# netocg/vae-decode-hdr

Hardware: NVIDIA B200
Metric: flux_vae_hdr_decode_megapixels_per_s (higher is better)
Workload: dtype fp16

## Files before the change

### vae_decode_hdr_b200/csrc/api.cu

```cuda
#include <stdarg.h>
#include <string.h>

#include <algorithm>
#include <functional>
#include <map>
#include <string>
#include <vector>

#include "engine.cuh"

namespace hdrvae {

static thread_local std::string g_last_error;
long long g_launch_count = 0;
void set_error(const char* fmt, ...) {
  char buf[1024];
  va_list ap;
  va_start(ap, fmt);
  vsnprintf(buf, sizeof buf, fmt, ap);
  va_end(ap);
  g_last_error = buf;
}

bool g_prof_on = false;
// ... 301 lines not shown
static bool x_is_16bit(hdrvae_ctx* ctx) {
  static int on = -1;
  if (on < 0) { const char* e = getenv("HDRVAE_X16"); on = (e && atoi(e) == 0) ? 0 : 1; }
  static int nin_on = -1;
  if (nin_on < 0) { const char* e = getenv("HDRVAE_FUSE_NIN"); nin_on = (e && atoi(e) == 0) ? 0 : 1; }
  return on && nin_on && !ctx->high && ctx->op_dtype == DT_F16 && ctx->conv_impl == HDRVAE_CONV_TCGEN05 && h_is_16bit(ctx);
}

static bool gn_is_fused(hdrvae_ctx* ctx, const PackedConv& pc, const ConvIO& io, int x_dtype, int H, int W) {
  static int on = -1;
  if (on < 0) {
    const char* e = getenv("HDRVAE_FUSE_GN");
    const char* g = getenv("HDRVAE_CTA_GROUP");
    on = ((e && atoi(e) == 0) || (g && atoi(g) == 1)) ? 0 : 1;
  }
  return on && x_is_16bit(ctx) && x_dtype == DT_F16 && pc.w_dtype == DT_F16 && pc.kmul == 1 && !pc.upsample && pc.ks == 3 &&
         pc.cout_pad >= 256 && pc.cin_pad % 64 == 0 && ctx->cta_group != 1 && io.x2 == nullptr && io.y_dtype == DT_F16 &&
         io.stats != nullptr && conv_takes_slab(pc, io, H, W, ctx->conv_impl);
}

static float* stats_ptr(hdrvae_ctx* ctx, DecState* st) {
  return ctx->conv_impl == HDRVAE_CONV_TCGEN05 ? reinterpret_cast<float*>(st->gn) : nullptr;
}

static int gn_before_conv(hdrvae_ctx* ctx, const void* x, const NormW& nw, const PackedConv& pc, ConvIO* io, DecState* st,
                          int B, int H, int W, cudaStream_t s, int x_dtype = DT_F32, float x_scale = 1.f) {
  if (gn_is_fused(ctx, pc, *io, x_dtype, H, W)) {
    char pname[64];
    snprintf(pname, sizeof pname, "groupnorm statistics C=%d @%dx%d", nw.C, B, H * W);
    ProfScope prof(pname, 0.0, 0.0, s);
    const int partials = st->pending;
    st->pending = 0;
    const float* scale = nullptr; const float* shift = nullptr;
// ... 10 lines not shown
  const int impl = ctx->conv_impl;
  const bool h16 = h_is_16bit(ctx);
  const int h_dt = h16 ? ctx->op_dtype : DT_F32;
  const float h_scale = h16 ? kRawOperandScale : 1.f;
  {
    ConvIO io; io.y = st->hbuf; io.stats = stats_ptr(ctx, st); io.stats_chunks = &st->pending;
    io.y_dtype = h_dt; io.y_scale = h_scale;
    HDRVAE_TRY(gn_before_conv(ctx, st->x, rw.n1, rw.c1, &io, st, B, H, W, s, st->x_dt, 1.f / st->x_scale));
    HDRVAE_TRY(run_conv(ctx, rw.c1, io, B, H, W, impl, s));
  }
  const bool x16 = st->x_dt != DT_F32;
  ConvIO io; io.stats = stats_ptr(ctx, st); io.stats_chunks = &st->pending;
  if (x16) { io.y_dtype = st->x_dt; io.y_scale = st->x_scale; }
  else if (rw.dual_out) { io.y2 = st->xa16; io.y2_dtype = ctx->op_dtype; io.y2_scale = kRawOperandScale; }
  if (rw.has_nin) {
    HDRVAE_TRY(run_gn(ctx, st->hbuf, h_dt, st->t, B, H * W, rw.n2, true, st, s, -1, 1.f / h_scale));
    io.x = st->t;
    if (nin_is_fused(ctx, rw, H, W)) {
      io.x2 = st->xb16; io.pc2 = &rw.nin_x16; io.bias = rw.bias_c2_nin; io.y = st->x;
      if (x16) {
        io.x2 = st->x; io.y = st->hbuf;
        HDRVAE_TRY(run_conv(ctx, rw.c2, io, B, H, W, impl, s));
        std::swap(st->x, st->hbuf);
        return 0;
      }
      return run_conv(ctx, rw.c2, io, B, H, W, impl, s);
    }
    HDRVAE_REQUIRE(!x16, "the 16-bit residual stream needs the fused shortcut");
    ConvIO sc; sc.x = st->xb16; sc.y = st->hbuf; sc.alpha = 1.0f / kRawOperandScale;
    HDRVAE_TRY(run_conv(ctx, rw.nin, sc, B, H, W, impl, s));
    io.y = st->hbuf; io.residual = st->hbuf;
    HDRVAE_TRY(run_conv(ctx, rw.c2, io, B, H, W, impl, s));
    std::swap(st->x, st->hbuf);
  } else {
    io.y = st->x; io.residual = st->x;
    if (x16) { io.res_dtype = st->x_dt; io.res_scale = 1.f / st->x_scale; }
    HDRVAE_TRY(gn_before_conv(ctx, st->hbuf, rw.n2, rw.c2, &io, st, B, H, W, s, h_dt, 1.f / h_scale));
    HDRVAE_TRY(run_conv(ctx, rw.c2, io, B, H, W, impl, s));
  }
  return 0;
// ... 145 lines not shown
    float* part = ksp > 1 ? reinterpret_cast<float*>(ksplit_scratch) : nullptr;
    return launch_attention_fused(q, 1024, (long long)pl.Tp * 1024, pl.T, q + 512, 1024, (long long)pl.Tp * 1024, pl.Tp, vt, pl.Tp,
                                  (long long)512 * pl.Tp, pl.T, o, (long long)pl.T * 512, pl.B, ctx->op_dtype, qk_alpha,
                                  attention_cta_group(ctx), ctx->num_sms, part, part ? part + (size_t)ksp * rows * 512 : nullptr,
                                  (long long)ksp * rows, s);
  }
  for (int b = 0; b < pl.B; ++b) {
    const uint16_t* q = reinterpret_cast<const uint16_t*>(qk) + (size_t)b * pl.Tp * 1024;
    HDRVAE_TRY(attention_rows(ctx, ws, pl.off_s, pl.off_p, pl.off_inv, pl.off_part, nullptr, 0, pl.s_rows, q, pl.T, q + 512,
                              reinterpret_cast<const uint16_t*>(vt) + (size_t)b * 512 * pl.Tp, pl.T, pl.Tp,
                              reinterpret_cast<uint16_t*>(o) + (size_t)b * pl.T * 512, qk_alpha, s));
  }
  return 0;
}

static int run_decoder(hdrvae_ctx* ctx, const float* latent, const Plan& pl, uint8_t* ws, void** features,
                       cudaStream_t s) {
  HDRVAE_REQUIRE(ctx->loaded, "hdrvae: weights not loaded");
  const int B = pl.B, impl = ctx->conv_impl, dt = ctx->op_dtype;
  int H = pl.h, W = pl.w;
  void* lat = ws + pl.off_lat;
  DecState st;
  st.xa16 = ws + pl.off_x16;
  st.xb16 = ws + pl.off_x16b;
  st.x = reinterpret_cast<float*>(ws + pl.off_x);
  st.hbuf = reinterpret_cast<float*>(ws + pl.off_h);
  st.t = ws + pl.off_t;
  st.gn = ws + pl.off_gn;
  st.gn_chunks = pl.gn_chunks;
  st.pending = 0;
  const bool x16 = x_is_16bit(ctx);
// ... 49 lines not shown
  HDRVAE_TRY(run_res(ctx, ctx->mid2, &st, B, H, W, s));
  for (int lvl = 3; lvl >= 0; --lvl) {
    for (int i = 0; i < 3; ++i) HDRVAE_TRY(run_res(ctx, ctx->up[lvl][i], &st, B, H, W, s));
    if (lvl != 0) {
      ConvIO io; io.x = st.xa16; io.y = st.hbuf; io.alpha = 1.0f / kRawOperandScale;
      if (x16) { io.x = st.x; io.y_dtype = st.x_dt; io.y_scale = st.x_scale; }
      else if (lvl <= 2) { io.y2 = st.xb16; io.y2_dtype = dt; io.y2_scale = kRawOperandScale; }
      io.stats = stats_ptr(ctx, &st); io.stats_chunks = &st.pending;
      HDRVAE_TRY(run_conv(ctx, ctx->upsample[lvl], io, B, H, W, impl, s));
      std::swap(st.x, st.hbuf);
      H *= 2; W *= 2;
    }
  }
  HDRVAE_TRY(run_gn(ctx, st.x, st.x_dt, st.t, B, H * W, ctx->norm_out, true, &st, s, ctx->high ? DT_F32 : -1, 1.f / st.x_scale));
  *features = st.t;
  return 0;
}

static int check_ws(const Plan& pl, void* ws, size_t bytes) {
  HDRVAE_REQUIRE(ws != nullptr && bytes >= pl.total, "hdrvae: workspace too small (%zu < %zu bytes)", bytes, pl.total);
  HDRVAE_REQUIRE((reinterpret_cast<uintptr_t>(ws) & 255) == 0, "hdrvae: workspace must be 256-byte aligned");
  return 0;
}


struct RowsPlan {
  int h, w, hl, world, T, Tl, Tp, s_rows, gn_chunks;
  size_t off_lat, off_x, off_h, off_t, off_xa, off_xb, off_gn, off_qk, off_v, off_vt, off_o, off_s, off_p, off_inv,
      off_part, off_epi, off_mail, total;
};
// ... 39 lines not shown

}

struct hdrvae_rows {
  hdrvae_ctx* ctx = nullptr;
  RowsPlan pl;
  int rank = 0, mode = 0;
  float factor = 1.f, ev = 1.f;
  uint8_t* ws = nullptr;
  const float* latent = nullptr;
  float* out = nullptr;
  struct Op { bool exchange; std::function<int(cudaStream_t)> fn; hdrvae_exchange ex; };
  std::vector<Op> ops;
  size_t pc = 0;
  float* x = nullptr; float* hbuf = nullptr;
  int H = 0, W = 0, pending = 0;
  uint8_t* peers[kRowsMaxRanks] = {};
  bool peers_set = false;
};

namespace hdrvae {

static void rows_compute(hdrvae_rows* st, std::function<int(cudaStream_t)> fn) {
  hdrvae_rows::Op op; op.exchange = false; op.fn = std::move(fn); memset(&op.ex, 0, sizeof op.ex);
  st->ops.push_back(std::move(op));
}
static void rows_exchange(hdrvae_rows* st, const hdrvae_exchange& ex) {
  hdrvae_rows::Op op; op.exchange = true; op.ex = ex;
  st->ops.push_back(std::move(op));
}
// ... 28 lines not shown
  hdrvae_exchange ex;
  memset(&ex, 0, sizeof ex);
  add_halo(st, &ex, slab_f32, H, W, C, eb);
  if (slab16 != nullptr) add_halo(st, &ex, slab16, H, W, C16, 2);
  ex.kind |= HDRVAE_EX_ALLREDUCE_F64;
  ex.allreduce_off = ws_off(st, gn_sums_ptr(gn, 1, 512, gn_chunks));
  ex.allreduce_count = 32 * 2;
  rows_exchange(st, ex);
  (void)ctx;
}

static void rows_gn(hdrvae_rows* st, const void* x_slab, const NormW& nw, bool silu, int H, int W, int x_dtype = DT_F32,
                    float in_scale = 1.f) {
  hdrvae_ctx* ctx = st->ctx;
  void* gn = st->ws + st->pl.off_gn;
  void* t = st->ws + st->pl.off_t;
  const int gn_chunks = st->pl.gn_chunks;
  const double count = (double)H * st->pl.world * (double)W * (double)(nw.C / 32);
  const NormW n = nw;
  rows_compute(st, [=](cudaStream_t s) {
    const long long slab = (long long)(H + 2) * W * n.C;
    HDRVAE_TRY(launch_gn_apply_from_sums(x_slab, x_dtype, slab, t, ctx->op_dtype, slab, 1, (H + 2) * W, n.C, n.gamma, n.beta,
                                         silu, gn, gn_chunks, count, s, in_scale));
    return zero_border_halos(st, t, H, W, n.C, 2, s);
  });
}

static void rows_res(hdrvae_rows* st, const ResW& rw, int H, int W) {
  hdrvae_ctx* ctx = st->ctx;
  void* t = st->ws + st->pl.off_t;
  void* xa = st->ws + st->pl.off_xa;
  void* xb = st->ws + st->pl.off_xb;
  float* stats = reinterpret_cast<float*>(st->ws + st->pl.off_gn);
  int* pending = &st->pending;
  float* x = st->x; float* hb = st->hbuf;
  const ResW* r = &rw;
  const bool h16 = h_is_16bit(ctx);
  const int h_dt = h16 ? ctx->op_dtype : DT_F32;
  const float h_scale = h16 ? kRawOperandScale : 1.f;
  const bool x16 = x_is_16bit(ctx);
  const int x_dt = x16 ? ctx->op_dtype : DT_F32;
  const float x_scale = x16 ? kRawOperandScale : 1.f;
  void* gn = st->ws + st->pl.off_gn;
  const int gn_chunks = st->pl.gn_chunks;
  const int y_lo = st->rank == 0 ? 0 : -1, y_hi = st->rank == st->pl.world - 1 ? H : H + 1;
// ... 1 lines not shown
  ConvIO probe1; probe1.y = hb; probe1.y_dtype = h_dt; probe1.stats = stats;
  const bool f1 = gn_is_fused(ctx, rw.c1, probe1, x_dt, H, W);
  if (!f1) rows_gn(st, x, rw.n1, true, H, W, x_dt, 1.f / x_scale);
  rows_compute(st, [=](cudaStream_t s) {
    ConvIO io; io.x = t; io.y = hb; io.stats = stats; io.stats_chunks = pending; io.x_pad = io.y_pad = 1;
    io.y_dtype = h_dt; io.y_scale = h_scale;
    if (f1) {
      HDRVAE_TRY(launch_gn_scale_shift_from_sums(1, r->n1.C, r->n1.gamma, r->n1.beta, gn, gn_chunks,
                                                 world_rows * (double)W * (double)(r->n1.C / 32), s, &io.xf_scale, &io.xf_shift));
      io.x = x; io.xf_in_scale = 1.f / x_scale; io.xf_y_lo = y_lo; io.xf_y_hi = y_hi;
    }
    return run_conv(ctx, r->c1, io, 1, H, W, HDRVAE_CONV_TCGEN05, s);
  });
  rows_stats_and_halo(st, hb, H, W, rw.c1.cout, nullptr, 0, h16 ? 2 : 4);
  const bool fused_nin = nin_is_fused(ctx, rw, H, W);
  float* out = (rw.has_nin && (!fused_nin || x16)) ? hb : x;
  ConvIO probe2; probe2.y = out; probe2.residual = rw.has_nin ? nullptr : out; probe2.y_dtype = x_dt; probe2.stats = stats;
  const bool f2 = !rw.has_nin && gn_is_fused(ctx, rw.c2, probe2, h_dt, H, W);
  if (!f2) rows_gn(st, hb, rw.n2, true, H, W, h_dt, 1.f / h_scale);
  rows_compute(st, [=](cudaStream_t s) {
    if (x16) {
      ConvIO io; io.x = t; io.y = out; io.stats = stats; io.stats_chunks = pending; io.x_pad = io.y_pad = 1;
      io.y_dtype = x_dt; io.y_scale = x_scale;
      if (fused_nin) { io.x2 = x; io.pc2 = &r->nin_x16; io.bias = r->bias_c2_nin; }
      else { io.residual = out; io.res_dtype = x_dt; io.res_scale = 1.f / x_scale; }
      if (f2) {
        HDRVAE_TRY(launch_gn_scale_shift_from_sums(1, r->n2.C, r->n2.gamma, r->n2.beta, gn, gn_chunks,
                                                   world_rows * (double)W * (double)(r->n2.C / 32), s, &io.xf_scale, &io.xf_shift));
        io.x = hb; io.xf_in_scale = 1.f / h_scale; io.xf_y_lo = y_lo; io.xf_y_hi = y_hi;
      }
      HDRVAE_TRY(run_conv(ctx, r->c2, io, 1, H, W, HDRVAE_CONV_TCGEN05, s));
      return zero_border_halos(st, out, H, W, r->c2.cout, 2, s);
    }
// ... 2 lines not shown
      io.x2 = xb; io.pc2 = &r->nin_x16; io.bias = r->bias_c2_nin;
      return run_conv(ctx, r->c2, io, 1, H, W, HDRVAE_CONV_TCGEN05, s);
    }
    if (r->has_nin) {
      ConvIO sc; sc.x = xb; sc.y = hb; sc.alpha = 1.0f / kRawOperandScale; sc.x_pad = sc.y_pad = 1;
      HDRVAE_TRY(run_conv(ctx, r->nin, sc, 1, H, W, HDRVAE_CONV_TCGEN05, s));
    }
    ConvIO io; io.x = t; io.y = out; io.residual = out; io.stats = stats; io.stats_chunks = pending; io.x_pad = io.y_pad = 1;
    if (r->dual_out) { io.y2 = xa; io.y2_dtype = ctx->op_dtype; io.y2_scale = kRawOperandScale; }
    HDRVAE_TRY(run_conv(ctx, r->c2, io, 1, H, W, HDRVAE_CONV_TCGEN05, s));
    if (r->dual_out) HDRVAE_TRY(zero_border_halos(st, xa, H, W, r->c2.cout, 2, s));
    return 0;
  });
  if (x16) rows_stats_and_halo(st, out, H, W, rw.c2.cout, nullptr, 0, 2);
  else rows_stats_and_halo(st, out, H, W, rw.c2.cout, rw.dual_out ? xa : nullptr, rw.c2.cout);
  if (rw.has_nin && (!fused_nin || x16)) std::swap(st->x, st->hbuf);
}

static int build_rows_program(hdrvae_rows* st) {
  hdrvae_ctx* ctx = st->ctx;
  const RowsPlan& pl = st->pl;
  const int dt = ctx->op_dtype;
  uint8_t* ws = st->ws;
  void* lat = ws + pl.off_lat;
  void* t = ws + pl.off_t;
  void* xa = ws + pl.off_xa;
  void* xb = ws + pl.off_xb;
  float* stats = reinterpret_cast<float*>(ws + pl.off_gn);
  int* pending = &st->pending;
  st->x = reinterpret_cast<float*>(ws + pl.off_x);
  st->hbuf = reinterpret_cast<float*>(ws + pl.off_h);
  int H = pl.hl, W = pl.w;
  const int rank = st->rank;
  const float* latent = st->latent;
  const bool x16 = x_is_16bit(ctx);
  const int x_dt = x16 ? dt : DT_F32;
  const float x_scale = x16 ? kRawOperandScale : 1.f;
  const int x_eb = x16 ? 2 : 4;

  {
    float* x = st->x;
    rows_compute(st, [=](cudaStream_t s) {
      HDRVAE_TRY(launch_latent_rows_to_nhwc(latent, lat, dt, 16, pl.h, pl.w, rank * pl.hl - 1, pl.hl + 2, 64, s));
      HDRVAE_TRY(gn_scratch_reset(stats, 1, pl.gn_chunks, s));
      ConvIO io; io.x = lat; io.y = x; io.stats = stats; io.stats_chunks = pending; io.x_pad = io.y_pad = 1;
      if (x16) { io.y_dtype = x_dt; io.y_scale = x_scale; }
      HDRVAE_TRY(run_conv(ctx, ctx->conv_in, io, 1, H, W, HDRVAE_CONV_TCGEN05, s));
      return x16 ? zero_border_halos(st, x, H, W, 512, 2, s) : 0;
    });
    rows_stats_and_halo(st, x, H, W, 512, nullptr, 0, x_eb);
  }
  rows_res(st, ctx->mid1, H, W);
  {
    uint16_t* qk = reinterpret_cast<uint16_t*>(ws + pl.off_qk);
    uint16_t* vb = reinterpret_cast<uint16_t*>(ws + pl.off_v);
    uint16_t* vt = reinterpret_cast<uint16_t*>(ws + pl.off_vt);
    uint16_t* o = reinterpret_cast<uint16_t*>(ws + pl.off_o);
    float* x = st->x;
    float* hscr = st->hbuf;
    const size_t hscr_bytes = (size_t)(8 * pl.hl + 2) * 8 * pl.w * 256 * 4;
    rows_gn(st, x, ctx->attn_norm, false, H, W, x_dt, 1.f / x_scale);
    rows_compute(st, [=](cudaStream_t s) {
      const uint16_t* tl = reinterpret_cast<const uint16_t*>(t) + (size_t)W * 512;
      if (pl.Tp != pl.T) {
        HDRVAE_CUDA_OK(cudaMemsetAsync(qk, 0, (size_t)pl.Tp * 1024 * 2, s));
        HDRVAE_CUDA_OK(cudaMemsetAsync(vt, 0, (size_t)512 * pl.Tp * 2, s));
      }
      HDRVAE_TRY(run_gemm(ctx, dt, tl, 512, pl.Tl, 512, ctx->qk.w[0], 512, 1024, 1024, qk + (size_t)rank * pl.Tl * 1024, 1024, dt,
                          ctx->qk.bias, false, 1.0f, nullptr, HDRVAE_CONV_TCGEN05, s));
      return run_gemm(ctx, dt, tl, 512, pl.Tl, 512, ctx->vproj.w[0], 512, 512, 512, vb + (size_t)rank * pl.Tl * 512, 512, dt,
                      ctx->vproj.bias, false, 1.0f, nullptr, HDRVAE_CONV_TCGEN05, s);
    });
    hdrvae_exchange ex;
    memset(&ex, 0, sizeof ex);
    ex.kind = HDRVAE_EX_ALLGATHER;
    ex.n_gather = 2;
// ... 22 lines not shown
        ConvIO io; io.x = xa; io.y = hb; io.alpha = 1.0f / kRawOperandScale; io.x_pad = io.y_pad = 1;
        if (x16) { io.x = xs; io.y_dtype = x_dt; io.y_scale = x_scale; }
        else if (lvl <= 2) { io.y2 = xb; io.y2_dtype = dt; io.y2_scale = kRawOperandScale; }
        io.stats = stats; io.stats_chunks = pending;
        HDRVAE_TRY(run_conv(ctx, *up, io, 1, Hc, Wc, HDRVAE_CONV_TCGEN05, s));
        return x16 ? zero_border_halos(st, hb, 2 * Hc, 2 * Wc, up->cout, 2, s) : 0;
      });
      H *= 2; W *= 2;
      rows_stats_and_halo(st, hb, H, W, up->cout, nullptr, 0, x_eb);
      std::swap(st->x, st->hbuf);
    }
  }
  {
    float* x = st->x;
    rows_gn(st, x, ctx->norm_out, true, H, W, x_dt, 1.f / x_scale);
    void* epi = ws + pl.off_epi;
    float* hscratch = st->hbuf;
    rows_compute(st, [=](cudaStream_t s) {
      return run_phase_a(ctx, t, 1, H, W, 1, hscratch, epi, s);
    });
    hdrvae_exchange ex;
    memset(&ex, 0, sizeof ex);
    ex.kind = HDRVAE_EX_RAW_STATS;
    ex.raw_stats_off = ws_off(st, epilogue_raw_stats_ptr(epi, 1, H, W));
    rows_exchange(st, ex);
    rows_compute(st, [=](cudaStream_t s) {
      return launch_epilogue_phase_b(1, H, W, st->mode, st->factor, st->ev, st->out, nullptr, epi, s);
    });
  }
  return 0;
// ... 248 lines not shown
  HDRVAE_CUDA_OK(cudaGraphLaunch(exec, s));
  return 0;
}

int hdrvae_decode_begin(hdrvae_ctx* ctx, const float* latent, int B, int h, int w, void* workspace, size_t ws_bytes,
                        void** raw_stats_dev, void* stream) {
  HDRVAE_REQUIRE(ctx != nullptr && latent != nullptr, "hdrvae_decode: null argument");
  HDRVAE_REQUIRE(B >= 1 && h >= 1 && w >= 1, "hdrvae_decode: empty latent batch [%d,16,%d,%d]", B, h, w);
  HDRVAE_CUDA_OK(cudaSetDevice(ctx->device));
  const Plan pl = make_plan(B, h, w, false, ctx->high, ctx->high || !attention_fused_enabled(ctx));
  HDRVAE_TRY(check_ws(pl, workspace, ws_bytes));
  uint8_t* ws = reinterpret_cast<uint8_t*>(workspace);
  cudaStream_t s = reinterpret_cast<cudaStream_t>(stream);
  auto body = [&](const float* lat) -> int {
    void* feat = nullptr;
    HDRVAE_TRY(run_decoder(ctx, lat, pl, ws, &feat, s));
    ProfScope prof("epilogue phase A (conv_out, max-pool, stats)", 2.0 * B * 64.0 * h * w * 3 * 1152, B * 64.0 * h * w * (256 + 24), s);
    return run_phase_a(ctx, feat, B, 8 * h, 8 * w, 0, reinterpret_cast<float*>(ws + pl.off_h), ws + pl.off_epi, s);
  };
  if (graphs_enabled(ctx, s)) {
    float* lat_in = reinterpret_cast<float*>(ws + pl.off_lat_in);
    HDRVAE_CUDA_OK(cudaMemcpyAsync(lat_in, latent, (size_t)B * 16 * pl.T * 4, cudaMemcpyDeviceToDevice, s));
    hdrvae_ctx::GraphEntry key{0, B, h, w, 0, ctx->conv_impl, ctx->cta_group, 0.f, 0.f, workspace, nullptr, 0};
    HDRVAE_TRY(run_segment(ctx, key, s, [&]() { return body(lat_in); }));
  } else {
    HDRVAE_TRY(body(latent));
  }
  if (raw_stats_dev != nullptr) *raw_stats_dev = epilogue_raw_stats_ptr(ws + pl.off_epi, B, 8 * h, 8 * w);
  return 0;
}

int hdrvae_decode_finish(hdrvae_ctx* ctx, int B, int h, int w, int mode, float expansion_factor, float ev_multiplier,
                         float* out_bhwc, hdrvae_stats* stats, void* workspace, size_t ws_bytes, void* stream) {
// ... 196 lines not shown
    if (e != cudaSuccess) { set_error("hdrvae_rows_end: %s", cudaGetErrorString(e)); r = -1; }
  }
  delete st;
  return r;
}

int hdrvae_decode_features(hdrvae_ctx* ctx, const float* latent, int B, int h, int w, void* features, void* workspace,
                           size_t ws_bytes, void* stream) {
  HDRVAE_REQUIRE(ctx != nullptr && latent != nullptr && features != nullptr, "hdrvae_decode_features: null argument");
  HDRVAE_REQUIRE(B >= 1 && h >= 1 && w >= 1, "hdrvae_decode_features: empty latent batch");
  HDRVAE_CUDA_OK(cudaSetDevice(ctx->device));
  const Plan pl = make_plan(B, h, w, false, ctx->high, ctx->high || !attention_fused_enabled(ctx));
  HDRVAE_TRY(check_ws(pl, workspace, ws_bytes));
  cudaStream_t s = reinterpret_cast<cudaStream_t>(stream);
  void* feat = nullptr;
  HDRVAE_TRY(run_decoder(ctx, latent, pl, reinterpret_cast<uint8_t*>(workspace), &feat, s));
  HDRVAE_CUDA_OK(cudaMemcpyAsync(features, feat, (size_t)B * 64 * h * w * 128 * (ctx->high ? 4 : 2), cudaMemcpyDeviceToDevice, s));
  return 0;
}

int hdrvae_epilogue_scratch_bytes(int B, int H, int W, size_t* bytes) {
  HDRVAE_REQUIRE(bytes != nullptr && B >= 1 && H >= 1 && W >= 1, "hdrvae_epilogue_scratch_bytes: bad argument");
  *bytes = epilogue_scratch_bytes(B, H, W);
  return 0;
}

int hdrvae_epilogue(hdrvae_ctx* ctx, const void* pre, int dtype, int B, int H, int W, const float* conv_w,
                    const float* conv_b, int mode, float expansion_factor, float ev_multiplier, float* out_bhwc,
                    hdrvae_stats* stats, float* dbg_post3, float* dbg_pre3, int32_t* dbg_argmax3, void* scratch,
                    size_t scratch_bytes, void* stream) {
  HDRVAE_REQUIRE(ctx != nullptr && pre != nullptr && conv_w != nullptr && conv_b != nullptr && out_bhwc != nullptr,
// ... 119 lines not shown
```

### vae_decode_hdr_b200/csrc/gemm_tc.cu

```cuda
#include "common.cuh"
#pragma nv_diag_suppress 128
#include "ptx.cuh"

#ifndef HDRVAE_SLAB_PITCH
#define HDRVAE_SLAB_PITCH 10
#endif

namespace hdrvae {

constexpr int kBlockM = 128;
constexpr int kRowBytes = 128;
constexpr int kABytes = kBlockM * kRowBytes;
constexpr int kEpilogueThreads = 256;
constexpr int kNumThreads = 128 + kEpilogueThreads;
constexpr int kRegsControl = 64, kRegsEpilogue = 216;

constexpr int kSmemLimit = 232448;
constexpr int kSmemFixed = 8 * 4096  + 256  +
                           1024 ;

constexpr int kSlabRows = 18, kSlabPitch = HDRVAE_SLAB_PITCH;
constexpr int kSlabBytes = kSlabRows * kSlabPitch * kRowBytes;
constexpr int kSlabBufBytes = (kSlabBytes + 1023) / 1024 * 1024;
template <int BLOCK_N, int CG, int KSUB, int SLAB = 0>
// ... 52 lines not shown
  EPI_GENERIC = 1,
  EPI_OUT16 = 2,
  EPI_RES = 4,
  EPI_OUT2 = 8,
  EPI_STATS = 16,
  EPI_ROWOPS = 32,
  EPI_LRELU = 64,
  EPI_RES2 = 128,
  EPI_ROWMAX = 256,
  EPI_EXPSUM = 512,
  EPI_RES16 = 1024,
};

constexpr int kXfWarps = 8;
constexpr int kXfThreads = kNumThreads + kXfWarps * 32;
constexpr int kRegsControlXf = 64, kRegsXf = 64, kRegsEpilogueXf = 144;

template <int BLOCK_N, bool kTf32, int CG, int EPI, int KSUB, int SLAB = 0, bool XF = false>
__global__ void __launch_bounds__(XF ? kXfThreads : kNumThreads, 1)
gemm_tc_kernel(const __grid_constant__ CUtensorMap tmA, const __grid_constant__ CUtensorMap tmB,
               const __grid_constant__ CUtensorMap tmA2, const __grid_constant__ CUtensorMap tmB2, const GemmParams p) {
  using Cfg = TcConfig<BLOCK_N, CG, KSUB, SLAB>;
  constexpr int kAT = Cfg::kATile;
  const uint32_t rank = CG == 2 ? ptx::cluster_ctarank() : 0u;
  constexpr int kStages = Cfg::kStages;
  constexpr int kActiveEpiWarps = BLOCK_N >= 64 ? 8 : 4;
  constexpr int kElemsPerRow = kTf32 ? 32 : 64;
  extern __shared__ uint8_t smem_raw[];
  uint8_t* smem = smem_raw + ((1024u - (ptx::smem_u32(smem_raw) & 1023u)) & 1023u);
  uint8_t* smem_a = smem;
  uint8_t* smem_b = SLAB ? smem : smem + kStages * KSUB * kAT;
// ... 39 lines not shown
  if (CG == 2) ptx::cluster_sync_all(); else __syncthreads();
  ptx::tc_fence_after_sync();
  const uint32_t tmem_base = *tmem_ptr_s;

  const int tiles_per_img = p.tiles_x * p.tiles_y;
  const int m_tiles = p.n_img * tiles_per_img;
  const int num_tiles = ((m_tiles + CG - 1) / CG) * p.n_tiles_n;
  const int w_first = blockIdx.x / CG, w_step = gridDim.x / CG;
  const int kb_per_tap = p.k_per_tap / kElemsPerRow;
  const int num_kb = p.ntaps * kb_per_tap;
  const int kb2_blocks = SLAB ? p.k2 / kElemsPerRow : 0;
  const int ntg = SLAB ? p.ntaps / SLAB : 0;
  constexpr bool xf = XF && SLAB > 0;

  const int num_groups = (num_kb + KSUB - 1) / KSUB;
  if (warp < 4 || warp >= 12) {
  if (!XF) ptx::reg_dec<kRegsControl>();
  else if (warp < 4) ptx::reg_dec<kRegsControlXf>();
  else ptx::reg_dec<kRegsXf>();
  if (warp == 0) {
    int stage = 0, ss = 0;
    uint32_t phase = 0, sphase = 0;
    int s_tile = w_first, s_kb = 0;
    auto issue_next_slab = [&]() {
      if (s_tile >= num_tiles) return;
      const int mt = (s_tile / p.n_tiles_n) * CG + (int)rank;
      const int img = mt / tiles_per_img;
      const int rem = mt - img * tiles_per_img;
      const int ty = rem / p.tiles_x;
      const int tx = rem - ty * p.tiles_x;
      const int x0 = tx * p.TW, y0 = ty * p.TH;
      ptx::mbar_wait(&slab_empty_bar[ss], sphase ^ 1);
      if (ptx::elect_one()) {
        uint8_t* sa = smem_slab + ss * Cfg::kSlabBuf;
// ... 207 lines not shown
            }
          }
          if (CG == 2) ptx::umma_commit_pair(&empty_bar[stage]); else ptx::umma_commit(&empty_bar[stage]);
          if (g == num_groups - 1) {
            if (CG == 2) ptx::umma_commit_pair(&tmem_full_bar[acc]); else ptx::umma_commit(&tmem_full_bar[acc]);
          }
        }
        __syncwarp();
        if (++stage == kStages) { stage = 0; phase ^= 1; }
      }
      if (++acc == 2) { acc = 0; acc_phase ^= 1; }
    }
    if (tim && blockIdx.x == 0 && lane == 0)
      printf("gemm_tc<%d,cg%d,epi%d,slab%d> issuer: %lld cycles, %d tiles x %d k-blocks; waited: accumulator %lld, slab %lld, B stage %lld\n",
             BLOCK_N, CG, EPI, SLAB, clock64() - t_begin, (num_tiles - w_first + w_step - 1) / w_step, num_kb, w_acc, w_slab, w_b);
  } else if (warp >= 12 && xf) {
    if constexpr (xf) {
      const int tl = (warp - 12) * 32 + lane;
      const int c = tl & 7, lg = tl >> 3;
      const uint32_t chunk_off = (uint32_t)((c ^ (lg & 7)) << 4);
      const int C = p.k_per_tap;
      const int y_hi = p.xf_y_hi;
      int ss = 0;
      uint32_t sphase = 0;
      const bool tim = (p.dbg & 32) != 0;
      long long w_land = 0, w_work = 0, tq = 0;
      for (int tile = w_first; tile < num_tiles; tile += w_step) {
        const int mt = (tile / p.n_tiles_n) * CG + (int)rank;
        const int img = mt / tiles_per_img;
        const int rem = mt - img * tiles_per_img;
        const int ty = rem / p.tiles_x;
        const int tx = rem - ty * p.tiles_x;
        const int x0 = tx * p.TW - 1, y0 = ty * p.TH - 1;
        const bool img_ok = img < p.n_img;
        for (int kb = 0; kb < kb_per_tap; ++kb) {
          float2 a2[4], b2[4];
#pragma unroll
          for (int e = 0; e < 4; ++e) {
            const int ch = kb * kElemsPerRow + c * 8 + 2 * e;
            const bool ok = img_ok && ch + 1 < C;
            a2[e].x = ok ? __ldg(p.xf_scale + (long long)img * C + ch) * p.xf_in_scale : 0.f;
            a2[e].y = ok ? __ldg(p.xf_scale + (long long)img * C + ch + 1) * p.xf_in_scale : 0.f;
            b2[e].x = ok ? __ldg(p.xf_shift + (long long)img * C + ch) : 0.f;
            b2[e].y = ok ? __ldg(p.xf_shift + (long long)img * C + ch + 1) : 0.f;
          }
          if (tim) tq = clock64();
          ptx::mbar_wait(&slab_full_bar[ss], sphase);
          if (tim) { const long long now = clock64(); w_land += now - tq; tq = now; }
          uint8_t* base = smem_slab + ss * Cfg::kSlabBuf + chunk_off;
          int r = lg / kSlabPitch, px = lg - r * kSlabPitch;
#pragma unroll 2
          for (int L = lg; L < kSlabRows * kSlabPitch; L += 32) {
            uint4* q = reinterpret_cast<uint4*>(base + L * kRowBytes);
            const int x = x0 + px, y = y0 + r;
            const bool inside = x >= 0 && x < p.W && y >= p.xf_y_lo && y < y_hi;
            uint4 v = *q;
            __half2* h = reinterpret_cast<__half2*>(&v);
#pragma unroll
            for (int e = 0; e < 4; ++e) {
              const float2 o = silu_nr2(f2_fma(__half22float2(h[e]), a2[e], b2[e]));
              h[e] = __floats2half2_rn(o.x, o.y);
            }
            if (!inside) v = make_uint4(0u, 0u, 0u, 0u);
            *q = v;
            px += 32 - 3 * kSlabPitch;
            r += 3;
            if (px >= kSlabPitch) { px -= kSlabPitch; ++r; }
          }
          ptx::fence_proxy_async();
          __syncwarp();
          if (lane == 0) {
            if (CG == 2) ptx::mbar_arrive_cluster(&slab_ready_bar[ss], 0);
            else ptx::mbar_arrive(&slab_ready_bar[ss]);
          }
          if (tim) w_work += clock64() - tq;
          if (++ss == Cfg::kSlabStages) { ss = 0; sphase ^= 1; }
        }
      }
      if (tim && blockIdx.x == 0 && warp == 12 && lane == 0)
        printf("gemm_tc<%d,cg%d,epi%d,slab%d> transform warp 0: waited for slabs to land %lld cycles, transformed them in %lld\n",
               BLOCK_N, CG, EPI, SLAB, w_land, w_work);
    }
// ... 653 lines not shown
      } else {
        epi = -1;
      }
    } else if (res16 && !p.round_tf32 && p.out_dtype == p.res_dtype && p.out2 == nullptr && !rowops && p.stats != nullptr) {
      epi = EPI_OUT16 | EPI_RES16 | EPI_STATS;
    } else {
      epi = -1;
    }
    if (p.row_mode != 0) {
      HDRVAE_REQUIRE(!n128 && p.tw_log2 == 7 && p.H == 1 && p.row_part != nullptr && p.ntaps == 1 && p.b_img_k_stride == 0,
                     "gemm_tc: the soft-max passes are row-major GEMMs with >= 256 columns");
      if (p.row_mode == 1) return launch_tc<256, false, 2, EPI_ROWMAX>(p, num_sms, stream);
      HDRVAE_REQUIRE(p.out_dtype != DT_F32 && p.bias != nullptr, "gemm_tc: soft-max pass 2 writes a 16-bit output and needs -max per row");
      return launch_tc<256, false, 2, EPI_OUT16 | EPI_EXPSUM>(p, num_sms, stream);
    }
    if (p.slab && n128 && p.ntaps == 9 && p.TW == 8 && p.TH == 16 && p.b_img_k_stride == 0) {
      if (epi == EPI_STATS) return launch_tc<128, false, 2, EPI_STATS, 3>(p, num_sms, stream);
      if (epi == (EPI_OUT16 | EPI_STATS)) return launch_tc<128, false, 2, EPI_OUT16 | EPI_STATS, 3>(p, num_sms, stream);
      if (epi == (EPI_RES | EPI_STATS)) return launch_tc<128, false, 2, EPI_RES | EPI_STATS, 3>(p, num_sms, stream);
      if (epi == (EPI_RES | EPI_OUT2 | EPI_STATS)) return launch_tc<128, false, 2, EPI_RES | EPI_OUT2 | EPI_STATS, 3>(p, num_sms, stream);
      if (epi == (EPI_OUT16 | EPI_RES16 | EPI_STATS)) return launch_tc<128, false, 2, EPI_OUT16 | EPI_RES16 | EPI_STATS, 3>(p, num_sms, stream);
      if (epi == 0) return launch_tc<128, false, 2, 0, 3>(p, num_sms, stream);
      if (epi == EPI_RES) return launch_tc<128, false, 2, EPI_RES, 3>(p, num_sms, stream);
    }
    if (p.slab && !n128 && p.ntaps == 4 && p.TW == 8 && p.TH == 16 && p.b_img_k_stride == 0) {
      if (epi == (EPI_OUT2 | EPI_STATS)) return launch_tc<256, false, 2, EPI_OUT2 | EPI_STATS, 1>(p, num_sms, stream);
      if (epi == EPI_STATS) return launch_tc<256, false, 2, EPI_STATS, 1>(p, num_sms, stream);
      if (epi == (EPI_OUT16 | EPI_STATS)) return launch_tc<256, false, 2, EPI_OUT16 | EPI_STATS, 1>(p, num_sms, stream);
      HDRVAE_REQUIRE(false, "gemm_tc: no slab build for this upsample epilogue (%d)", epi);
    }
    if (p.xf_scale != nullptr) {
      HDRVAE_REQUIRE(p.slab && !n128 && p.ntaps == 9 && p.TW == 8 && p.TH == 16 && p.b_img_k_stride == 0 && p.k2 == 0,
                     "gemm_tc: the fused GroupNorm exists for the 256-column 3x3 slab convs");
      if (epi == (EPI_OUT16 | EPI_STATS)) return launch_tc<256, false, 2, EPI_OUT16 | EPI_STATS, 1, true>(p, num_sms, stream);
      if (epi == (EPI_OUT16 | EPI_RES16 | EPI_STATS)) return launch_tc<256, false, 2, EPI_OUT16 | EPI_RES16 | EPI_STATS, 1, true>(p, num_sms, stream);
      HDRVAE_REQUIRE(false, "gemm_tc: no fused-GroupNorm build for this epilogue (%d)", epi);
    }
    if (p.slab && !n128 && p.ntaps == 9 && p.TW == 8 && p.TH == 16 && p.b_img_k_stride == 0) {
      if (epi == EPI_STATS) return launch_tc<256, false, 2, EPI_STATS, 1>(p, num_sms, stream);
      if (epi == (EPI_OUT16 | EPI_STATS)) return launch_tc<256, false, 2, EPI_OUT16 | EPI_STATS, 1>(p, num_sms, stream);
      if (epi == (EPI_RES | EPI_STATS)) return launch_tc<256, false, 2, EPI_RES | EPI_STATS, 1>(p, num_sms, stream);
      if (epi == (EPI_RES | EPI_OUT2 | EPI_STATS)) return launch_tc<256, false, 2, EPI_RES | EPI_OUT2 | EPI_STATS, 1>(p, num_sms, stream);
      if (epi == (EPI_OUT16 | EPI_RES16 | EPI_STATS)) return launch_tc<256, false, 2, EPI_OUT16 | EPI_RES16 | EPI_STATS, 1>(p, num_sms, stream);
    }
#define HDRVAE_EPI_CASE(E)                                                                       \
    case E:                                                                                      \
      return n128 ? launch_tc<128, false, 2, E>(p, num_sms, stream) : launch_tc<256, false, 2, E>(p, num_sms, stream);
    switch (epi) {
      HDRVAE_EPI_CASE(0)
      HDRVAE_EPI_CASE(EPI_RES)
      HDRVAE_EPI_CASE(EPI_STATS)
// ... 21 lines not shown
```

Baseline: 117.9.

## Extend fused GroupNorm to shortcut and 128-column convs, add interior slab fast path

Fused GroupNorm+SiLU-in-the-conv-prologue now also covers convs with a fused 1x1 shortcut (x2) and 128-column (n128) convs. This removes the standalone GroupNorm pass and its round trip through the t buffer in residual blocks with a channel-change shortcut. The t buffer is rotated to serve as an output, and the spare x buffer is passed to phase A as scratch. The transform warps gain an unrolled interior-tile path that skips per-pixel bounds logic, and register budgets are rebalanced between the transform and epilogue warps, at the cost of more template instantiations and register pressure.

```diff
diff --git a/vae_decode_hdr_b200/csrc/api.cu b/vae_decode_hdr_b200/csrc/api.cu
--- a/vae_decode_hdr_b200/csrc/api.cu
+++ b/vae_decode_hdr_b200/csrc/api.cu
@@ -339,9 +339,10 @@
     const char* g = getenv("HDRVAE_CTA_GROUP");
     on = ((e && atoi(e) == 0) || (g && atoi(g) == 1)) ? 0 : 1;
   }
+  const bool cols_ok = pc.cout_pad >= 256 || pc.cin_pad >= 256 || io.x2 != nullptr;
   return on && x_is_16bit(ctx) && x_dtype == DT_F16 && pc.w_dtype == DT_F16 && pc.kmul == 1 && !pc.upsample && pc.ks == 3 &&
-         pc.cout_pad >= 256 && pc.cin_pad % 64 == 0 && ctx->cta_group != 1 && io.x2 == nullptr && io.y_dtype == DT_F16 &&
-         io.stats != nullptr && conv_takes_slab(pc, io, H, W, ctx->conv_impl);
+         cols_ok && pc.cin_pad % 64 == 0 && ctx->cta_group != 1 && io.y_dtype == DT_F16 && io.stats != nullptr &&
+         conv_takes_slab(pc, io, H, W, ctx->conv_impl);
 }
 
 static float* stats_ptr(hdrvae_ctx* ctx, DecState* st) {
@@ -382,16 +383,20 @@
   if (x16) { io.y_dtype = st->x_dt; io.y_scale = st->x_scale; }
   else if (rw.dual_out) { io.y2 = st->xa16; io.y2_dtype = ctx->op_dtype; io.y2_scale = kRawOperandScale; }
   if (rw.has_nin) {
+    if (nin_is_fused(ctx, rw, H, W) && x16) {
+      io.x2 = st->x; io.pc2 = &rw.nin_x16; io.bias = rw.bias_c2_nin;
+      const bool gn_fused = gn_is_fused(ctx, rw.c2, io, h_dt, H, W);
+      HDRVAE_TRY(gn_before_conv(ctx, st->hbuf, rw.n2, rw.c2, &io, st, B, H, W, s, h_dt, 1.f / h_scale));
+      io.y = gn_fused ? st->t : st->hbuf;
+      HDRVAE_TRY(run_conv(ctx, rw.c2, io, B, H, W, impl, s));
+      if (gn_fused) { st->t = st->x; st->x = static_cast<float*>(io.y); }
+      else std::swap(st->x, st->hbuf);
+      return 0;
+    }
     HDRVAE_TRY(run_gn(ctx, st->hbuf, h_dt, st->t, B, H * W, rw.n2, true, st, s, -1, 1.f / h_scale));
     io.x = st->t;
     if (nin_is_fused(ctx, rw, H, W)) {
       io.x2 = st->xb16; io.pc2 = &rw.nin_x16; io.bias = rw.bias_c2_nin; io.y = st->x;
-      if (x16) {
-        io.x2 = st->x; io.y = st->hbuf;
-        HDRVAE_TRY(run_conv(ctx, rw.c2, io, B, H, W, impl, s));
-        std::swap(st->x, st->hbuf);
-        return 0;
-      }
       return run_conv(ctx, rw.c2, io, B, H, W, impl, s);
     }
     HDRVAE_REQUIRE(!x16, "the 16-bit residual stream needs the fused shortcut");
@@ -567,7 +572,7 @@
   return 0;
 }
 
-static int run_decoder(hdrvae_ctx* ctx, const float* latent, const Plan& pl, uint8_t* ws, void** features,
+static int run_decoder(hdrvae_ctx* ctx, const float* latent, const Plan& pl, uint8_t* ws, void** features, float** spare,
                        cudaStream_t s) {
   HDRVAE_REQUIRE(ctx->loaded, "hdrvae: weights not loaded");
   const int B = pl.B, impl = ctx->conv_impl, dt = ctx->op_dtype;
@@ -647,6 +652,7 @@
   }
   HDRVAE_TRY(run_gn(ctx, st.x, st.x_dt, st.t, B, H * W, ctx->norm_out, true, &st, s, ctx->high ? DT_F32 : -1, 1.f / st.x_scale));
   *features = st.t;
+  if (spare != nullptr) *spare = st.x;
   return 0;
 }
 
@@ -716,6 +722,7 @@
   std::vector<Op> ops;
   size_t pc = 0;
   float* x = nullptr; float* hbuf = nullptr;
+  void* t = nullptr;
   int H = 0, W = 0, pending = 0;
   uint8_t* peers[kRowsMaxRanks] = {};
   bool peers_set = false;
@@ -774,7 +781,7 @@
                     float in_scale = 1.f) {
   hdrvae_ctx* ctx = st->ctx;
   void* gn = st->ws + st->pl.off_gn;
-  void* t = st->ws + st->pl.off_t;
+  void* t = st->t;
   const int gn_chunks = st->pl.gn_chunks;
   const double count = (double)H * st->pl.world * (double)W * (double)(nw.C / 32);
   const NormW n = nw;
@@ -788,7 +795,7 @@
 
 static void rows_res(hdrvae_rows* st, const ResW& rw, int H, int W) {
   hdrvae_ctx* ctx = st->ctx;
-  void* t = st->ws + st->pl.off_t;
+  void* t = st->t;
   void* xa = st->ws + st->pl.off_xa;
   void* xb = st->ws + st->pl.off_xb;
   float* stats = reinterpret_cast<float*>(st->ws + st->pl.off_gn);
@@ -820,9 +827,12 @@
   });
   rows_stats_and_halo(st, hb, H, W, rw.c1.cout, nullptr, 0, h16 ? 2 : 4);
   const bool fused_nin = nin_is_fused(ctx, rw, H, W);
-  float* out = (rw.has_nin && (!fused_nin || x16)) ? hb : x;
-  ConvIO probe2; probe2.y = out; probe2.residual = rw.has_nin ? nullptr : out; probe2.y_dtype = x_dt; probe2.stats = stats;
-  const bool f2 = !rw.has_nin && gn_is_fused(ctx, rw.c2, probe2, h_dt, H, W);
+  ConvIO probe2; probe2.y_dtype = x_dt; probe2.stats = stats;
+  if (fused_nin && x16) probe2.x2 = x;
+  if (!rw.has_nin) probe2.residual = x;
+  const bool f2 = (!rw.has_nin || (fused_nin && x16)) && gn_is_fused(ctx, rw.c2, probe2, h_dt, H, W);
+  const bool rotate_t = rw.has_nin && f2;
+  void* out = rotate_t ? t : (rw.has_nin && (!fused_nin || x16)) ? static_cast<void*>(hb) : static_cast<void*>(x);
   if (!f2) rows_gn(st, hb, rw.n2, true, H, W, h_dt, 1.f / h_scale);
   rows_compute(st, [=](cudaStream_t s) {
     if (x16) {
@@ -855,7 +865,8 @@
   });
   if (x16) rows_stats_and_halo(st, out, H, W, rw.c2.cout, nullptr, 0, 2);
   else rows_stats_and_halo(st, out, H, W, rw.c2.cout, rw.dual_out ? xa : nullptr, rw.c2.cout);
-  if (rw.has_nin && (!fused_nin || x16)) std::swap(st->x, st->hbuf);
+  if (rotate_t) { st->t = st->x; st->x = static_cast<float*>(out); }
+  else if (rw.has_nin && (!fused_nin || x16)) std::swap(st->x, st->hbuf);
 }
 
 static int build_rows_program(hdrvae_rows* st) {
@@ -864,13 +875,13 @@
   const int dt = ctx->op_dtype;
   uint8_t* ws = st->ws;
   void* lat = ws + pl.off_lat;
-  void* t = ws + pl.off_t;
   void* xa = ws + pl.off_xa;
   void* xb = ws + pl.off_xb;
   float* stats = reinterpret_cast<float*>(ws + pl.off_gn);
   int* pending = &st->pending;
   st->x = reinterpret_cast<float*>(ws + pl.off_x);
   st->hbuf = reinterpret_cast<float*>(ws + pl.off_h);
+  st->t = ws + pl.off_t;
   int H = pl.hl, W = pl.w;
   const int rank = st->rank;
   const float* latent = st->latent;
@@ -901,6 +912,7 @@
     float* hscr = st->hbuf;
     const size_t hscr_bytes = (size_t)(8 * pl.hl + 2) * 8 * pl.w * 256 * 4;
     rows_gn(st, x, ctx->attn_norm, false, H, W, x_dt, 1.f / x_scale);
+    void* t = st->t;
     rows_compute(st, [=](cudaStream_t s) {
       const uint16_t* tl = reinterpret_cast<const uint16_t*>(t) + (size_t)W * 512;
       if (pl.Tp != pl.T) {
@@ -953,6 +965,7 @@
   {
     float* x = st->x;
     rows_gn(st, x, ctx->norm_out, true, H, W, x_dt, 1.f / x_scale);
+    void* t = st->t;
     void* epi = ws + pl.off_epi;
     float* hscratch = st->hbuf;
     rows_compute(st, [=](cudaStream_t s) {
@@ -1231,9 +1244,10 @@
   cudaStream_t s = reinterpret_cast<cudaStream_t>(stream);
   auto body = [&](const float* lat) -> int {
     void* feat = nullptr;
-    HDRVAE_TRY(run_decoder(ctx, lat, pl, ws, &feat, s));
+    float* conv8 = nullptr;
+    HDRVAE_TRY(run_decoder(ctx, lat, pl, ws, &feat, &conv8, s));
     ProfScope prof("epilogue phase A (conv_out, max-pool, stats)", 2.0 * B * 64.0 * h * w * 3 * 1152, B * 64.0 * h * w * (256 + 24), s);
-    return run_phase_a(ctx, feat, B, 8 * h, 8 * w, 0, reinterpret_cast<float*>(ws + pl.off_h), ws + pl.off_epi, s);
+    return run_phase_a(ctx, feat, B, 8 * h, 8 * w, 0, conv8, ws + pl.off_epi, s);
   };
   if (graphs_enabled(ctx, s)) {
     float* lat_in = reinterpret_cast<float*>(ws + pl.off_lat_in);
@@ -1460,7 +1474,7 @@
   HDRVAE_TRY(check_ws(pl, workspace, ws_bytes));
   cudaStream_t s = reinterpret_cast<cudaStream_t>(stream);
   void* feat = nullptr;
-  HDRVAE_TRY(run_decoder(ctx, latent, pl, reinterpret_cast<uint8_t*>(workspace), &feat, s));
+  HDRVAE_TRY(run_decoder(ctx, latent, pl, reinterpret_cast<uint8_t*>(workspace), &feat, nullptr, s));
   HDRVAE_CUDA_OK(cudaMemcpyAsync(features, feat, (size_t)B * 64 * h * w * 128 * (ctx->high ? 4 : 2), cudaMemcpyDeviceToDevice, s));
   return 0;
 }
diff --git a/vae_decode_hdr_b200/csrc/gemm_tc.cu b/vae_decode_hdr_b200/csrc/gemm_tc.cu
--- a/vae_decode_hdr_b200/csrc/gemm_tc.cu
+++ b/vae_decode_hdr_b200/csrc/gemm_tc.cu
@@ -90,7 +90,7 @@
 
 constexpr int kXfWarps = 8;
 constexpr int kXfThreads = kNumThreads + kXfWarps * 32;
-constexpr int kRegsControlXf = 64, kRegsXf = 64, kRegsEpilogueXf = 144;
+constexpr int kRegsControlXf = 64, kRegsXf = 72, kRegsEpilogueXf = 136;
 
 template <int BLOCK_N, bool kTf32, int CG, int EPI, int KSUB, int SLAB = 0, bool XF = false>
 __global__ void __launch_bounds__(XF ? kXfThreads : kNumThreads, 1)
@@ -160,10 +160,8 @@
   constexpr bool xf = XF && SLAB > 0;
 
   const int num_groups = (num_kb + KSUB - 1) / KSUB;
-  if (warp < 4 || warp >= 12) {
-  if (!XF) ptx::reg_dec<kRegsControl>();
-  else if (warp < 4) ptx::reg_dec<kRegsControlXf>();
-  else ptx::reg_dec<kRegsXf>();
+  if (warp < 4) {
+  ptx::reg_dec<XF ? kRegsControlXf : kRegsControl>();
   if (warp == 0) {
     int stage = 0, ss = 0;
     uint32_t phase = 0, sphase = 0;
@@ -401,13 +399,18 @@
     if (tim && blockIdx.x == 0 && lane == 0)
       printf("gemm_tc<%d,cg%d,epi%d,slab%d> issuer: %lld cycles, %d tiles x %d k-blocks; waited: accumulator %lld, slab %lld, B stage %lld\n",
              BLOCK_N, CG, EPI, SLAB, clock64() - t_begin, (num_tiles - w_first + w_step - 1) / w_step, num_kb, w_acc, w_slab, w_b);
-  } else if (warp >= 12 && xf) {
+  }
+  } else if (warp >= 12) {
+  if (XF) ptx::reg_dec<kRegsXf>();
+  {
     if constexpr (xf) {
       const int tl = (warp - 12) * 32 + lane;
       const int c = tl & 7, lg = tl >> 3;
       const uint32_t chunk_off = (uint32_t)((c ^ (lg & 7)) << 4);
       const int C = p.k_per_tap;
       const int y_hi = p.xf_y_hi;
+      constexpr int kXfLines = (kSlabRows * kSlabPitch + 31) / 32;
+      const bool last_line = lg + 32 * (kXfLines - 1) < kSlabRows * kSlabPitch;
       int ss = 0;
       uint32_t sphase = 0;
       const bool tim = (p.dbg & 32) != 0;
@@ -420,6 +423,7 @@
         const int tx = rem - ty * p.tiles_x;
         const int x0 = tx * p.TW - 1, y0 = ty * p.TH - 1;
         const bool img_ok = img < p.n_img;
+        const bool interior = img_ok && x0 >= 0 && x0 + kSlabPitch <= p.W && y0 >= p.xf_y_lo && y0 + kSlabRows <= y_hi;
         for (int kb = 0; kb < kb_per_tap; ++kb) {
           float2 a2[4], b2[4];
 #pragma unroll
@@ -435,6 +439,24 @@
           ptx::mbar_wait(&slab_full_bar[ss], sphase);
           if (tim) { const long long now = clock64(); w_land += now - tq; tq = now; }
           uint8_t* base = smem_slab + ss * Cfg::kSlabBuf + chunk_off;
+          if (interior) {
+            uint4 v[kXfLines];
+#pragma unroll
+            for (int i = 0; i < kXfLines; ++i)
+              if (i + 1 < kXfLines || last_line) v[i] = *reinterpret_cast<const uint4*>(base + (lg + 32 * i) * kRowBytes);
+#pragma unroll
+            for (int i = 0; i < kXfLines; ++i) {
+              __half2* h = reinterpret_cast<__half2*>(&v[i]);
+#pragma unroll
+              for (int e = 0; e < 4; ++e) {
+                const float2 o = silu_nr2(f2_fma(__half22float2(h[e]), a2[e], b2[e]));
+                h[e] = __floats2half2_rn(o.x, o.y);
+              }
+            }
+#pragma unroll
+            for (int i = 0; i < kXfLines; ++i)
+              if (i + 1 < kXfLines || last_line) *reinterpret_cast<uint4*>(base + (lg + 32 * i) * kRowBytes) = v[i];
+          } else {
           int r = lg / kSlabPitch, px = lg - r * kSlabPitch;
 #pragma unroll 2
           for (int L = lg; L < kSlabRows * kSlabPitch; L += 32) {
@@ -453,6 +475,7 @@
             px += 32 - 3 * kSlabPitch;
             r += 3;
             if (px >= kSlabPitch) { px -= kSlabPitch; ++r; }
+          }
           }
           ptx::fence_proxy_async();
           __syncwarp();
@@ -1136,6 +1159,17 @@
       HDRVAE_REQUIRE(p.out_dtype != DT_F32 && p.bias != nullptr, "gemm_tc: soft-max pass 2 writes a 16-bit output and needs -max per row");
       return launch_tc<256, false, 2, EPI_OUT16 | EPI_EXPSUM>(p, num_sms, stream);
     }
+    if (p.xf_scale != nullptr) {
+      HDRVAE_REQUIRE(p.slab && p.ntaps == 9 && p.TW == 8 && p.TH == 16 && p.b_img_k_stride == 0,
+                     "gemm_tc: the fused GroupNorm exists for the 3x3 slab convs");
+      if (n128) {
+        if (epi == (EPI_OUT16 | EPI_STATS)) return launch_tc<128, false, 2, EPI_OUT16 | EPI_STATS, 3, true>(p, num_sms, stream);
+      } else {
+        if (epi == (EPI_OUT16 | EPI_STATS)) return launch_tc<256, false, 2, EPI_OUT16 | EPI_STATS, 1, true>(p, num_sms, stream);
+        if (epi == (EPI_OUT16 | EPI_RES16 | EPI_STATS)) return launch_tc<256, false, 2, EPI_OUT16 | EPI_RES16 | EPI_STATS, 1, true>(p, num_sms, stream);
+      }
+      HDRVAE_REQUIRE(false, "gemm_tc: no fused-GroupNorm build for this epilogue (%d, %d columns)", epi, p.n_cols);
+    }
     if (p.slab && n128 && p.ntaps == 9 && p.TW == 8 && p.TH == 16 && p.b_img_k_stride == 0) {
       if (epi == EPI_STATS) return launch_tc<128, false, 2, EPI_STATS, 3>(p, num_sms, stream);
       if (epi == (EPI_OUT16 | EPI_STATS)) return launch_tc<128, false, 2, EPI_OUT16 | EPI_STATS, 3>(p, num_sms, stream);
@@ -1150,13 +1184,6 @@
       if (epi == EPI_STATS) return launch_tc<256, false, 2, EPI_STATS, 1>(p, num_sms, stream);
       if (epi == (EPI_OUT16 | EPI_STATS)) return launch_tc<256, false, 2, EPI_OUT16 | EPI_STATS, 1>(p, num_sms, stream);
       HDRVAE_REQUIRE(false, "gemm_tc: no slab build for this upsample epilogue (%d)", epi);
-    }
-    if (p.xf_scale != nullptr) {
-      HDRVAE_REQUIRE(p.slab && !n128 && p.ntaps == 9 && p.TW == 8 && p.TH == 16 && p.b_img_k_stride == 0 && p.k2 == 0,
-                     "gemm_tc: the fused GroupNorm exists for the 256-column 3x3 slab convs");
-      if (epi == (EPI_OUT16 | EPI_STATS)) return launch_tc<256, false, 2, EPI_OUT16 | EPI_STATS, 1, true>(p, num_sms, stream);
-      if (epi == (EPI_OUT16 | EPI_RES16 | EPI_STATS)) return launch_tc<256, false, 2, EPI_OUT16 | EPI_RES16 | EPI_STATS, 1, true>(p, num_sms, stream);
-      HDRVAE_REQUIRE(false, "gemm_tc: no fused-GroupNorm build for this epilogue (%d)", epi);
     }
     if (p.slab && !n128 && p.ntaps == 9 && p.TW == 8 && p.TH == 16 && p.b_img_k_stride == 0) {
       if (epi == EPI_STATS) return launch_tc<256, false, 2, EPI_STATS, 1>(p, num_sms, stream);
```

Result: no change. 118.9 (median of 6 runs) (+0.9%).
